# Baverne/VAE-CYCLEGAN-Implementation

Hardware: AMD Instinct MI355X
Metric: train images/sec (256x256 VAE-CycleGAN step) (higher is better)
Workload: dtype f32; 1 GPU; cyclevaegan unpaired, 3x256x256 synthetic summer<->winter, per-GPU batch 8, latent 64 (BASELINE.json configs[3]/[4]); per_gpu_batch=8, global_batch=8, image_size=256, latent_dim=64, parallelism=dp1, init=random (reference init statistics)

## Files before the change

vae-cyclegan-implementation_amd/csrc/conv_igemm.hip:

```cpp
#include "vcg_common.h"
#ifdef VCG_STAMP
#include <stdlib.h>
#endif

struct ConvP {
  const float* a;
  const float* b;
  const float* bias;
  float* out;
  int N, H, W, Cin, Cout, KH, KW, stride, pad, reflect, ups, act;
  int Hl, Wl, Ho, Wo, M, K;
  int cin4, cout4, cout_log;
  FastDiv fd_howo, fd_wo, fd_cin4, fd_cout4, fd_kw, fd_cin;
  int Hc, Wc, Mc, NB;
  FastDiv fd_hcwc, fd_wc;
  int ktiles_total, sk_len, sk_units, sk_ntn, sk_bm_shift, sk_bn_shift;
  int sk_ntr_pb;
  FastDiv fd_sklen;
  int ksplit, kt_per;
  float* slab;
  int adjoint;
  int src_pitch;
  uint32_t a_bytes, b_bytes;
  int dbl_mirror;
// ... 1891 lines not shown
typedef void (*ConvKernel)(ConvP);
struct KernelRef { ConvKernel fn; const char* name; };

static KernelRef fwd_fp32_kernel(const Tile& t, bool single_level) {
  const char* const name = "k_conv_fwd<fp32 MFMA>";
  if (t.bm == 128 && t.bn == 128 && single_level) return {k_conv_fwd<128, 128, 2, false>, name};
  if (t.bn == 32) return {k_conv_fwd<128, 32, 1>, name};
  if (t.bm == 128 && t.bn == 128) return {k_conv_fwd<128, 128>, name};
  if (t.bm == 128 && t.bn == 64) return {k_conv_fwd<128, 64>, name};
  if (t.bm == 64 && t.bn == 128) return {k_conv_fwd<64, 128>, name};
  return {k_conv_fwd<64, 64>, name};
}
static void launch_fwd_tile(const Tile& t, const KernelRef& k, const ConvP& p, hipStream_t st) {
  dim3 grid((p.M + t.bm - 1) / t.bm, (p.Cout + t.bn - 1) / t.bn, p.nbatch * p.ksplit);
  VcgProfScope prof(k.name, 2.0 * p.M * (double)p.K * p.Cout * p.nbatch, st);
  hipLaunchKernelGGL(k.fn, grid, dim3(256), 0, st, p);
}

static ConvGeom gemm_geom(int rows, int K, int Ncols) {
  ConvGeom g = {};
  g.N = 1; g.H = 1; g.W = rows; g.Cin = K; g.Cout = Ncols; g.KH = g.KW = 1; g.stride = 1; g.pad = 0; g.reflect = 0;
  g.ups = 1; g.act = VCG_ACT_NONE; g.cin_log = K; g.cout_log = Ncols;
  g.Hl = 1; g.Wl = rows; g.Ho = 1; g.Wo = rows; g.M = rows; g.K = K; g.taps = 1;
  return g;
}
int vcg_gemm_batched(const float* A, const float* B, float* C, int rows, int K, int Ncols, int batches, hipStream_t st) {
  ConvP p; fill_params(gemm_geom(rows, K, Ncols), p);
  p.a = A; p.b = B; p.bias = nullptr; p.out = C;
  if (set_extents(p, (unsigned long long)rows * K * 4, (unsigned long long)K * Ncols * 4,
                  "vcg_gemm_batched: operand extents must stay below 2 GiB per batch")) return -1;
  p.nbatch = batches; p.a_bstride = (uint32_t)((size_t)rows * K); p.b_bstride = (uint32_t)((size_t)K * Ncols);
  p.out_bstride = (size_t)rows * Ncols;
  VCG_CHECK_ARG((unsigned long long)rows * K * (unsigned long long)batches < (1ull << 32), "vcg_gemm_batched: batch stride overflow");
  const Tile t = gemm_plan(rows, Ncols, (K + BK - 1) / BK, false, batches, false, K <= 2048);
  launch_fwd_tile(t, fwd_fp32_kernel(t, K <= 2048), p, st);
  VCG_LAUNCH_CHECK("vcg_gemm_batched");
  return 0;
}

int vcg_fwd_launch(const ConvGeom& g, const float* x, const float* wf, float* y, hipStream_t st) {
  ConvP p; fill_params(g, p);
  p.a = x; p.b = wf; p.bias = nullptr; p.out = y; p.act = VCG_ACT_NONE;
  if (set_extents(p, (unsigned long long)g.N * g.H * g.W * g.Cin * 4, (unsigned long long)g.K * g.Cout * 4,
                  "vcg_conv_fwd: tensor extents must stay below 2 GiB")) return -1;
  const Tile t = gemm_plan(g.M, g.Cout, (g.K + BK - 1) / BK, false, 1, true);
  launch_fwd_tile(t, fwd_fp32_kernel(t, false), p, st);
  VCG_LAUNCH_CHECK("vcg_conv_fwd(raw)");
  return 0;
}

extern "C" size_t vcg_pack_weight_floats(const int32_t* cd) {
  ConvGeom g;
  if (vcg_conv_geom(cd, &g, "vcg_pack_weight_floats")) return 0;
  return pack_layout(g).total;
}

extern "C" int vcg_pack_weight(const float* w_oihw, float* wf, const int32_t* cd, void* stream) {
  ConvGeom g;
  if (vcg_conv_geom(cd, &g, "vcg_pack_weight")) return -1;
  VCG_CHECK_ARG(w_oihw && wf, "vcg_pack_weight: null pointer");
  const PackLayout L = pack_layout(g);
  hipStream_t st = (hipStream_t)stream;
  const VcgAmaxOut aw = vcg_amax_new(st);
  if (vcg_absmax_launch(w_oihw, (size_t)g.cout_log * g.cin_log * g.ups * g.ups * g.KH * g.KW, aw, st)) return -2;
  const VcgAmax amax_w = vcg_amax_in(aw);
  ConvP p; fill_params(g, p);
  p.amax_b = amax_w;
  if (L.wkd > L.wk && vcg_thin_fold_pack(g, w_oihw, wf + L.wk, amax_w, st)) return -2;
  if (L.wft > L.wkd && vcg_thin_fold_dgrad_pack(g, w_oihw, wf + L.wkd, amax_w, st)) return -2;
  if (L.wfd > L.wft) {
    const size_t tot = (size_t)g.Cout * ((g.K + 31) / 32) * 8;
    int blocks = (int)((tot + 255) / 256); if (blocks > 8192) blocks = 8192;
    hipLaunchKernelGGL(k_pack_planes<false>, dim3(blocks), dim3(256), 0, st, w_oihw, (unsigned short*)(wf + L.wft), p, g.cin_log,
                       g.cout_log);
    VCG_LAUNCH_CHECK("vcg_pack_weight(WFT planes)");
  }
  if (L.hdr > L.wfd) {
    const size_t tot = (size_t)g.K * (g.Cout / 4);
    int blocks = (int)((tot + 255) / 256); if (blocks > 8192) blocks = 8192;
    hipLaunchKernelGGL(k_pack_planes<true>, dim3(blocks), dim3(256), 0, st, w_oihw, (unsigned short*)(wf + L.wfd), p, g.cin_log,
                       g.cout_log);
    VCG_LAUNCH_CHECK("vcg_pack_weight(WFD planes)");
  }
  if (L.ud > L.u && vcg_wino_weight(g, w_oihw, wf + L.u, amax_w, st)) return -2;
  if (L.wk > L.ud && vcg_wino_weight_dgrad(g, w_oihw, wf + L.ud, amax_w, st)) return -2;
  uint32_t* const hdr = (uint32_t*)(wf + L.hdr);
  if (cd[VCG_CD_PACK_FLAGS] & 1) {
    ConvP q = p; q.K = 0; q.Cout = 0;
    hipLaunchKernelGGL(k_pack_weight, dim3(1), dim3(64), 0, st, w_oihw, wf, q, g.cin_log, g.cout_log, hdr);
    VCG_LAUNCH_CHECK("vcg_pack_weight(header)");
    return 0;
  }
  size_t total = (size_t)g.K * g.Cout;
  const size_t lds = (size_t)g.taps * 8 * 33 * sizeof(float);
  if (total < (1u << 20) || lds > 64 * 1024) {
    int blocks = (int)((total + 255) / 256); if (blocks > 4096) blocks = 4096;
    hipLaunchKernelGGL(k_pack_weight, dim3(blocks), dim3(256), 0, st, w_oihw, wf, p, g.cin_log, g.cout_log, hdr);
  } else {
    hipLaunchKernelGGL(k_pack_weight_t, dim3((g.Cout + 31) / 32, (g.Cin + 7) / 8), dim3(256), lds, st, w_oihw, wf, p, g.cin_log,
                       g.cout_log, hdr);
  }
  VCG_LAUNCH_CHECK("vcg_pack_weight");
  return 0;
}

static int ew_grid(size_t work) {
  size_t b = (work + 255) / 256;
  if (b > 2048) b = 2048;
  return b < 1 ? 1 : (int)b;
}

static KernelRef fwd_kernel(const FwdPlan& pl) {
  if (pl.path == FWD_FP32) return fwd_fp32_kernel(pl.t, pl.single_level);
  if (pl.t.bn == 128) return {k_conv_fwd_split<128>, "k_conv_fwd_split<128>"};
  return {k_conv_fwd_split<64>, "k_conv_fwd_split<64>"};
}

static uint64_t take_fwd_hints() {
  const uint64_t x_handle = vcg_take_hint_x(); (void)vcg_take_hint_dy();
  return x_handle;
}

static int conv_fwd_impl(const ConvGeom& g, const FwdPlan& pl, uint64_t x_handle, const float* x, const float* wf, const float* bias,
                         float* y, void* ws, size_t ws_bytes, void* stream, double* in_part, const VcgInStatsOut* stats,
                         float* saved = nullptr, const VcgPre* pre = nullptr) {
  VCG_CHECK_ARG(x && wf && y, "vcg_conv_fwd: null pointer");
  if (pre && pre->mean)
    VCG_CHECK_ARG(pl.pre_ok, "vcg_conv_fwd_in_pre: this geometry has no normalising gather (ask vcg_conv_pre_ok first)");
  const PackLayout L = pack_layout(g);
  const void* const w_amax = wf + L.hdr;
  hipStream_t st = (hipStream_t)stream;
  auto finalize = [&]() {
    return in_part ? vcg_in_finalize(in_part, stats->mean, stats->rstd, g.N, stats->HW, g.Cout, pl.stats_nchunk, stats->eps, st) : 0;
  };
  if (pl.path == FWD_THIN_FOLD) return vcg_thin_fold_fwd(g, x, wf + L.wk, w_amax, bias, y, ws, ws_bytes, st, x_handle);
  if (pl.path == FWD_THIN) return vcg_thin_fwd(g, x, wf, bias, y, st);
  if (pl.path == FWD_THININ) return vcg_thinin_fwd(g, x, wf, w_amax, bias, y, in_part, st, x_handle) ? -2 : finalize();
  if (pl.path == FWD_WINO) return vcg_wino_fwd(g, x, wf + L.u, w_amax, bias, y, ws, ws_bytes, st, in_part, stats, saved, x_handle, pre);
  if (pl.path == FWD_SLAB) return vcg_slab_fwd(g, x, wf + L.wft, (L.wfd - L.wft) * 4, w_amax, bias, y, in_part, stats, st, x_handle);
  ConvP p; fill_params(g, p);
  if (in_part) { p.in_part = in_part; p.in_nchunk = pl.stats_nchunk; }
  p.a = x; p.b = wf; p.bias = bias; p.out = y;
  if (set_extents(p, (unsigned long long)g.N * g.H * g.W * g.Cin * 4, (unsigned long long)g.K * g.Cout * 4,
                  "vcg_conv_fwd: tensor extents must stay below 2 GiB")) return -1;
  const int nsplit = pl.t.nsplit;
  if (nsplit > 1) {
    VCG_CHECK_ARG(ws && ws_bytes >= pl.ws, "vcg_conv_fwd: workspace too small (%zu)", ws_bytes);
    p.ksplit = nsplit; p.kt_per = pl.t.kt_per; p.slab = (float*)ws;
  }
  if (pl.path == FWD_SPLIT) {
    p.b = wf + L.wft;
    p.b_bytes = (uint32_t)((L.wfd - L.wft) * 4);
    if (vcg_operand_amax(x, (size_t)g.N * g.H * g.W * g.Cin, x_handle, 0, st, &p.amax_a)) return -2;
    p.amax_b = vcg_amax_stored(w_amax);
  }
  launch_fwd_tile(pl.t, fwd_kernel(pl), p, st);
  if (nsplit > 1)
    hipLaunchKernelGGL(k_splitk_finish, dim3(ew_grid((size_t)g.M * g.Cout / 4)), dim3(256), 0, st, (const float*)ws, bias,
                       y, (size_t)g.M, g.Cout, nsplit, g.cout_log, g.act);
  VCG_LAUNCH_CHECK("vcg_conv_fwd");
  return finalize();
}

extern "C" size_t vcg_conv_fwd_workspace(const int32_t* cd) {
  ConvGeom g;
  if (vcg_conv_geom(cd, &g, "vcg_conv_fwd_workspace")) return 0;
  return plan_fwd(g).ws;
}
// ... 375 lines not shown
```

vae-cyclegan-implementation_amd/csrc/conv_wino.hip:

```cpp
#include "vcg_common.h"
#ifdef VCG_STAMP
#include <stdlib.h>
#endif

#define WINO_U_SHIFT 2
#define WINO_V_SHIFT 2
int vcg_gemm_planes_batched(const void* APlanes, const void* BtPlanes, float* C, int rows, int K, int N, int batches, const VcgAmax& amax_a,
                            const VcgAmax& amax_b, hipStream_t st, uint32_t* amax_a_keep);

struct WinoP {
  const float* x;
  const float* m;
  const float* bias;
  float* y;
  int N, H, W, Cin, Cout, Hl, Wl, ups, reflect, act, cout_log;
  int th, tw, T, Kc;
  int off;
  FastDiv fd_k4, fd_tw, fd_thtw, fd_c4, fd_co4;
  unsigned long long* amax_slot;
  uint32_t amax_gen;
  VcgAmax amax_x;
  unsigned short* vplanes;
  const float* pre_mean;
  const float* pre_rstd;
// ... 120 lines not shown
        }
      }
  }
}

__global__ __launch_bounds__(256) void k_wino_out_stats(WinoP p, double* __restrict__ part, NormPlan pl) {
  __shared__ double r1[256 * 4];
  __shared__ double r2[256 * 4];
  const int tc = threadIdx.x % pl.TC, tp = threadIdx.x / pl.TC;
  const int c4 = blockIdx.z * pl.TC + tc;
  const int n = blockIdx.y;
  const int tiles = p.th * p.tw;
  const int pb = blockIdx.x * pl.chunk;
  int pe = pb + pl.chunk;
  if (pe > tiles) pe = tiles;
  const size_t plane = (size_t)p.T * p.Cout;
  double s1[4] = {0.0, 0.0, 0.0, 0.0}, s2[4] = {0.0, 0.0, 0.0, 0.0};
  if (c4 * 4 < p.Cout) {
    const int co = c4 * 4;
    float4 bv = make_float4(0.f, 0.f, 0.f, 0.f);
    if (p.bias) {
      if (co + 0 < p.cout_log) bv.x = p.bias[co + 0];
      if (co + 1 < p.cout_log) bv.y = p.bias[co + 1];
      if (co + 2 < p.cout_log) bv.z = p.bias[co + 2];
      if (co + 3 < p.cout_log) bv.w = p.bias[co + 3];
    }
    for (int tl = pb + tp; tl < pe; tl += pl.TP) {
      const int ty = tl / p.tw, tx = tl - ty * p.tw;
      const size_t t = (size_t)n * tiles + tl;
      const float* mb = p.m + t * p.Cout + co;
      float4 a0[4], a1[4];
#pragma unroll
      for (int b = 0; b < 4; ++b) {
        const float4 m0 = *reinterpret_cast<const float4*>(mb + (size_t)(0 + b) * plane);
        const float4 m1 = *reinterpret_cast<const float4*>(mb + (size_t)(4 + b) * plane);
        const float4 m2 = *reinterpret_cast<const float4*>(mb + (size_t)(8 + b) * plane);
        const float4 m3 = *reinterpret_cast<const float4*>(mb + (size_t)(12 + b) * plane);
        a0[b] = f4sum(f4sum(m0, m1), m2);
        a1[b] = f4sub(f4sub(m1, m2), m3);
      }
      float4 y[2][2];
      y[0][0] = f4sum(f4sum(a0[0], a0[1]), a0[2]);
      y[0][1] = f4sub(f4sub(a0[1], a0[2]), a0[3]);
      y[1][0] = f4sum(f4sum(a1[0], a1[1]), a1[2]);
      y[1][1] = f4sub(f4sub(a1[1], a1[2]), a1[3]);
#pragma unroll
      for (int r = 0; r < 2; ++r)
#pragma unroll
        for (int q = 0; q < 2; ++q) {
          float4 o = y[r][q];
          o.x = act_apply(o.x + bv.x, p.act); o.y = act_apply(o.y + bv.y, p.act);
          o.z = act_apply(o.z + bv.z, p.act); o.w = act_apply(o.w + bv.w, p.act);
          *reinterpret_cast<float4*>(p.y + (((size_t)n * p.Hl + 2 * ty + r) * p.Wl + 2 * tx + q) * p.Cout + co) = o;
          s1[0] += (double)o.x; s2[0] += (double)o.x * (double)o.x;
          s1[1] += (double)o.y; s2[1] += (double)o.y * (double)o.y;
          s1[2] += (double)o.z; s2[2] += (double)o.z * (double)o.z;
          s1[3] += (double)o.w; s2[3] += (double)o.w * (double)o.w;
        }
    }
  }
#pragma unroll
  for (int e = 0; e < 4; ++e) {
    r1[threadIdx.x * 4 + e] = s1[e];
    r2[threadIdx.x * 4 + e] = s2[e];
  }
  __syncthreads();
  if (tp == 0 && c4 * 4 < p.Cout) {
    for (int k = 1; k < pl.TP; ++k) {
#pragma unroll
      for (int e = 0; e < 4; ++e) {
        s1[e] += r1[(k * pl.TC + tc) * 4 + e];
        s2[e] += r2[(k * pl.TC + tc) * 4 + e];
      }
    }
    double* o = part + (((size_t)n * pl.nchunk + blockIdx.x) * p.Cout + c4 * 4) * 2;
#pragma unroll
    for (int e = 0; e < 4; ++e) {
      o[2 * e] = s1[e];
      o[2 * e + 1] = s2[e];
    }
  }
}

template <bool DGRAD>
__global__ __launch_bounds__(256) void k_wino_weight_planes(const float* __restrict__ w, unsigned short* __restrict__ up, int Cin,
                                                            int Cout, int ups, int cin_log, int cout_log, VcgAmax amax) {
  float sc, inv;
  vcg_scale_of(vcg_amax_bits(amax), amax.shift, sc, inv);
  const int U2 = ups * ups, Kc = U2 * Cin;
  const int NR = DGRAD ? Kc : Cout, KD = DGRAD ? Cout : Kc;
  const size_t total = (size_t)NR * (KD / 4);
  for (size_t idx = (size_t)blockIdx.x * blockDim.x + threadIdx.x; idx < total; idx += (size_t)gridDim.x * blockDim.x) {
    const int n = (int)(idx / (KD / 4)), kk = (int)(idx - (size_t)n * (KD / 4)) * 4;
    float t[16][4];
#pragma unroll
    for (int e = 0; e < 4; ++e) {
      const int co = DGRAD ? kk + e : n, k = DGRAD ? n : kk + e;
      const int ph = k / Cin, c = k - ph * Cin;
      const bool ok = co < cout_log && c < cin_log;
      const float* wp = w + ((size_t)co * (cin_log * U2) + (size_t)c * U2 + ph) * 9;
      float g[3][3];
#pragma unroll
      for (int a = 0; a < 3; ++a)
#pragma unroll
        for (int b = 0; b < 3; ++b) g[a][b] = ok ? (DGRAD ? wp[(2 - a) * 3 + (2 - b)] : wp[a * 3 + b]) : 0.f;
      float h[4][3];
#pragma unroll
      for (int b = 0; b < 3; ++b) {
        h[0][b] = g[0][b];
        h[1][b] = 0.5f * (g[0][b] + g[1][b] + g[2][b]);
        h[2][b] = 0.5f * (g[0][b] - g[1][b] + g[2][b]);
        h[3][b] = g[2][b];
      }
#pragma unroll
      for (int a = 0; a < 4; ++a) {
        t[a * 4 + 0][e] = h[a][0];
        t[a * 4 + 1][e] = 0.5f * (h[a][0] + h[a][1] + h[a][2]);
        t[a * 4 + 2][e] = 0.5f * (h[a][0] - h[a][1] + h[a][2]);
        t[a * 4 + 3][e] = h[a][2];
      }
    }
#pragma unroll
    for (int xi = 0; xi < 16; ++xi) {
      uint2 hh, ll;
      split4h(make_float4(t[xi][0], t[xi][1], t[xi][2], t[xi][3]), inv, hh, ll);
      unsigned short* o = up + (((size_t)xi * NR + n) * (KD / 32) + kk / 32) * VCG_PBLK + (kk & 31);
      *reinterpret_cast<uint2*>(o) = hh;
      *reinterpret_cast<uint2*>(o + 32) = ll;
    }
  }
}

__global__ __launch_bounds__(256) void k_wino_out_pad(const float* __restrict__ m, float* __restrict__ dxp, WinoP p) {
  const uint32_t k4n = (uint32_t)p.Kc / 4;
  const size_t total = (size_t)p.T * k4n;
  const size_t plane = (size_t)p.T * p.Kc;
  const int Hp = 2 * p.th, Wp = 2 * p.tw;
  for (size_t idx = (size_t)blockIdx.x * blockDim.x + threadIdx.x; idx < total; idx += (size_t)gridDim.x * blockDim.x) {
    const uint32_t t = (uint32_t)(idx / k4n);
    const int k = (int)(idx - (size_t)t * k4n) * 4;
    const uint32_t n = fd_div(t, p.fd_thtw);
    const uint32_t rem = t - n * (uint32_t)(p.th * p.tw);
    const uint32_t ty = fd_div(rem, p.fd_tw);
    const int tx = (int)(rem - ty * (uint32_t)p.tw);
    const float* mb = m + (size_t)t * p.Kc + k;
    float4 s0[4], s1[4];
#pragma unroll
    for (int b = 0; b < 4; ++b) {
      const float4 m0 = *reinterpret_cast<const float4*>(mb + (size_t)(0 + b) * plane);
      const float4 m1 = *reinterpret_cast<const float4*>(mb + (size_t)(4 + b) * plane);
      const float4 m2 = *reinterpret_cast<const float4*>(mb + (size_t)(8 + b) * plane);
      const float4 m3 = *reinterpret_cast<const float4*>(mb + (size_t)(12 + b) * plane);
      s0[b] = f4sum(f4sum(m0, m1), m2);
      s1[b] = f4sub(f4sub(m1, m2), m3);
    }
    float* o = dxp + (((size_t)n * Hp + 2 * ty) * Wp + 2 * tx) * p.Kc + k;
    *reinterpret_cast<float4*>(o) = f4sum(f4sum(s0[0], s0[1]), s0[2]);
    *reinterpret_cast<float4*>(o + p.Kc) = f4sub(f4sub(s0[1], s0[2]), s0[3]);
    *reinterpret_cast<float4*>(o + (size_t)Wp * p.Kc) = f4sum(f4sum(s1[0], s1[1]), s1[2]);
    *reinterpret_cast<float4*>(o + (size_t)Wp * p.Kc + p.Kc) = f4sub(f4sub(s1[1], s1[2]), s1[3]);
  }
}

__device__ __forceinline__ float4 wino_out_elem(const float* __restrict__ mb, size_t plane, int rr, int cc) {
  float4 acc = make_float4(0.f, 0.f, 0.f, 0.f);
#pragma unroll
  for (int i = 0; i < 3; ++i) {
    const int xi_r = rr + i;
    const float sr = (rr == 1 && i > 0) ? -1.f : 1.f;
#pragma unroll
    for (int j = 0; j < 3; ++j) {
      const int xi_c = cc + j;
      const float sc = (cc == 1 && j > 0) ? -1.f : 1.f;
      const float4 v = *reinterpret_cast<const float4*>(mb + (size_t)(xi_r * 4 + xi_c) * plane);
      const float sg = sr * sc;
      acc.x += sg * v.x; acc.y += sg * v.y; acc.z += sg * v.z; acc.w += sg * v.w;
    }
  }
  return acc;
}
__global__ __launch_bounds__(256) void k_wino_out_fold(const float* __restrict__ m, float* __restrict__ dx, WinoP p, int Hl, int Wl,
                                                       int Cin, int ups, int reflect) {
  const uint32_t k4n = (uint32_t)p.Kc / 4;
  const size_t total = (size_t)p.T * k4n;
  const size_t plane = (size_t)p.T * p.Kc;
  const int W = Wl * ups;
  for (size_t idx = (size_t)blockIdx.x * blockDim.x + threadIdx.x; idx < total; idx += (size_t)gridDim.x * blockDim.x) {
    const uint32_t t = (uint32_t)(idx / k4n);
    const int k = (int)(idx - (size_t)t * k4n) * 4;
    const uint32_t n = fd_div(t, p.fd_thtw);
    const uint32_t rem = t - n * (uint32_t)(p.th * p.tw);
    const int ty = (int)fd_div(rem, p.fd_tw);
    const int tx = (int)(rem - (uint32_t)ty * (uint32_t)p.tw);
    const float* mb = m + (size_t)t * p.Kc + k;
    float4 s0[4], s1[4];
#pragma unroll
    for (int b = 0; b < 4; ++b) {
      const float4 m0 = *reinterpret_cast<const float4*>(mb + (size_t)(0 + b) * plane);
      const float4 m1 = *reinterpret_cast<const float4*>(mb + (size_t)(4 + b) * plane);
      const float4 m2 = *reinterpret_cast<const float4*>(mb + (size_t)(8 + b) * plane);
      const float4 m3 = *reinterpret_cast<const float4*>(mb + (size_t)(12 + b) * plane);
      s0[b] = f4sum(f4sum(m0, m1), m2);
      s1[b] = f4sub(f4sub(m1, m2), m3);
    }
    float4 o[2][2];
    o[0][0] = f4sum(f4sum(s0[0], s0[1]), s0[2]);
    o[0][1] = f4sub(f4sub(s0[1], s0[2]), s0[3]);
    o[1][0] = f4sum(f4sum(s1[0], s1[1]), s1[2]);
    o[1][1] = f4sub(f4sub(s1[1], s1[2]), s1[3]);
    const int ph = k / Cin, c = k - ph * Cin;
    const int pi = ph >> 1, pj = ph & 1;
// ... 167 lines not shown
    e[2][s] = f4sub(d[2][s], d[1][s]);
    e[3][s] = f4sub(d[1][s], d[3][s]);
  }
  const uint32_t k = k4 * 4;
  const size_t KB = (size_t)p.Kc / 32;
  const int TB = p.T / 32;
#pragma unroll
  for (int a = 0; a < 4; ++a) {
    const float4 o[4] = {f4sub(e[a][0], e[a][2]), f4sum(e[a][1], e[a][2]), f4sub(e[a][2], e[a][1]), f4sub(e[a][1], e[a][3])};
    if (p.vplanes) {
      unsigned short* vb = p.vplanes + ((size_t)t * KB + k / 32) * VCG_PBLK + (k & 31);
      const size_t plane = (size_t)p.T * KB * VCG_PBLK;
#pragma unroll
      for (int b = 0; b < 4; ++b) {
        uint2 h, l;
        split4h(o[b], inv, h, l);
        unsigned short* w = vb + (size_t)(a * 4 + b) * plane;
        *reinterpret_cast<uint2*>(w) = h;
        *reinterpret_cast<uint2*>(w + 32) = l;
      }
    }
    if (vt) wino_tr_store(sh, o, inv, tl, q, vt + (size_t)(a * 4) * p.Kc * TB * VCG_PBLK, (size_t)p.Kc * TB * VCG_PBLK, (size_t)blockIdx.y * 32, TB, (int)blockIdx.x);
  }
}
__global__ __launch_bounds__(256) void k_wino_dy_tr(const float* __restrict__ dy, unsigned short* __restrict__ dmt, WinoP p) {
  __shared__ __attribute__((aligned(16))) unsigned short sh[4 * 2 * 32 * WT_PITCH];
  float sc, inv;
  vcg_scale_of(vcg_amax_bits(p.amax_x), p.amax_x.shift, sc, inv);
  const int tl = threadIdx.x >> 3, q = threadIdx.x & 7;
  const uint32_t t = blockIdx.x * 32 + tl;
  const int co = ((int)blockIdx.y * 8 + q) * 4;
  const uint32_t n = fd_div(t, p.fd_thtw);
  const uint32_t rem = t - n * (uint32_t)(p.th * p.tw);
  const uint32_t ty = fd_div(rem, p.fd_tw);
  const int tx = (int)(rem - ty * (uint32_t)p.tw);
  const float* base = dy + (((size_t)n * p.Hl + 2 * ty) * p.Wl + 2 * tx) * p.Cout + co;
  const float4 y00 = *reinterpret_cast<const float4*>(base);
  const float4 y01 = *reinterpret_cast<const float4*>(base + p.Cout);
  const float4 y10 = *reinterpret_cast<const float4*>(base + (size_t)p.Wl * p.Cout);
  const float4 y11 = *reinterpret_cast<const float4*>(base + (size_t)p.Wl * p.Cout + p.Cout);
  const float4 zero = make_float4(0.f, 0.f, 0.f, 0.f);
  float4 z[4][2];
  z[0][0] = y00;              z[0][1] = y01;
  z[1][0] = f4sum(y00, y10);  z[1][1] = f4sum(y01, y11);
  z[2][0] = f4sub(y00, y10);  z[2][1] = f4sub(y01, y11);
  z[3][0] = f4sub(zero, y10); z[3][1] = f4sub(zero, y11);
  const int TB = p.T / 32;
#pragma unroll
  for (int a = 0; a < 4; ++a) {
    const float4 o[4] = {z[a][0], f4sum(z[a][0], z[a][1]), f4sub(z[a][0], z[a][1]), f4sub(zero, z[a][1])};
    wino_tr_store(sh, o, inv, tl, q, dmt + (size_t)(a * 4) * p.Cout * TB * VCG_PBLK, (size_t)p.Cout * TB * VCG_PBLK, (size_t)blockIdx.y * 32, TB, (int)blockIdx.x);
  }
}

static int wino_blocks(size_t work) {
  size_t b = (work + 255) / 256;
  if (b > 8192) b = 8192;
  return b < 1 ? 1 : (int)b;
}

bool vcg_wino_weight_ok(const ConvGeom& g) {
  return g.KH == 3 && g.KW == 3 && g.stride == 1 && g.pad == 1 && g.ups * g.ups * g.Cin >= 128 && g.Cout >= 64 &&
         g.Cin % 4 == 0 && g.Cout % 64 == 0 && (g.ups * g.ups * g.Cin) % 64 == 0;
}
static bool wino_map_ok(const ConvGeom& g) {
  if (!vcg_wino_weight_ok(g)) return false;
#ifdef VCG_STAMP
  if (getenv("VCG_NO_WINOGRAD")) return false;
#endif
  return !(g.Ho < 4 || g.Wo < 4 || (g.Ho & 1) || (g.Wo & 1));
}
bool vcg_wino_fwd_ok(const ConvGeom& g) {
  if (!wino_map_ok(g)) return false;
  const unsigned long long T = (unsigned long long)g.N * (g.Ho / 2) * (g.Wo / 2);
  const unsigned long long Kc = (unsigned long long)g.ups * g.ups * g.Cin;
  if (Kc * g.Cout < (unsigned long long)kWinoGateFwd * (Kc + g.Cout)) return false;
  return T * Kc * 4 < (1ull << 31) && T * g.Cout * 4 < (1ull << 31) && T * Kc * 16 < (1ull << 32);
}
size_t vcg_wino_weight_floats(const ConvGeom& g) { return (size_t)16 * g.ups * g.ups * g.Cin * g.Cout * VCG_NP / 2; }
size_t vcg_wino_fwd_workspace(const ConvGeom& g) {
  const size_t T = (size_t)g.N * (g.Ho / 2) * (g.Wo / 2);
  return (size_t)16 * T * ((size_t)g.ups * g.ups * g.Cin + g.Cout) * sizeof(float) + 512;
}
int vcg_wino_weight(const ConvGeom& g, const float* w_oihw, float* u, const VcgAmax& amax_w, hipStream_t st) {
  const size_t total = (size_t)g.ups * g.ups * g.Cin * g.Cout / 4;
  VcgAmax au = amax_w; au.shift += WINO_U_SHIFT;
  hipLaunchKernelGGL(k_wino_weight_planes<false>, dim3(wino_blocks(total)), dim3(256), 0, st, w_oihw, (unsigned short*)u, g.Cin, g.Cout,
                     g.ups, g.cin_log, g.cout_log, au);
  VCG_LAUNCH_CHECK("vcg_wino_weight");
  return 0;
}

static WinoP wino_params(const ConvGeom& g) {
  WinoP p = {};
  p.x = nullptr; p.m = nullptr; p.bias = nullptr; p.y = nullptr;
  p.N = g.N; p.H = g.H; p.W = g.W; p.Cin = g.Cin; p.Cout = g.Cout; p.Hl = g.Hl; p.Wl = g.Wl; p.ups = g.ups;
  p.reflect = g.reflect; p.act = g.act; p.cout_log = g.cout_log;
  p.th = g.Ho / 2; p.tw = g.Wo / 2; p.T = g.N * p.th * p.tw; p.Kc = g.ups * g.ups * g.Cin;
  p.fd_k4 = make_fastdiv((uint32_t)p.Kc / 4); p.fd_tw = make_fastdiv((uint32_t)p.tw);
  p.fd_thtw = make_fastdiv((uint32_t)(p.th * p.tw)); p.fd_c4 = make_fastdiv((uint32_t)g.Cin / 4);
  p.fd_co4 = make_fastdiv((uint32_t)g.Cout / 4);
  p.off = 1;
  p.amax_slot = nullptr; p.amax_gen = 0;
  p.amax_x = vcg_amax_const(0); p.vplanes = nullptr;
  p.pre_mean = nullptr; p.pre_rstd = nullptr; p.pre_act = VCG_ACT_NONE;
  return p;
}

bool vcg_wino_wgrad_ok(const ConvGeom& g) {
  const long long kc = (long long)g.ups * g.ups * g.Cin;
  return vcg_wino_fwd_ok(g) && kc % 128 == 0 && kc * g.Cout >= kWinoGateWgrad * (kc + g.Cout);
}
bool vcg_wino_wgrad_tr_ok(const ConvGeom& g) {
  if (!vcg_wino_wgrad_ok(g)) return false;
  const long long kc = (long long)g.ups * g.ups * g.Cin, T = (long long)g.N * (g.Ho / 2) * (g.Wo / 2);
  return T % 32 == 0 && kc % 32 == 0 && g.Cout % 128 == 0 && kc >= 256 && ((kc + 255) / 256) * (g.Cout / 128) * 16 >= 192 &&
         16 * kc * T * VCG_NP < (1ll << 32) && 16 * (long long)g.Cout * T * VCG_NP < (1ll << 32);
}
size_t vcg_wino_wgrad_workspace(const ConvGeom& g) {
  const int T = g.N * (g.Ho / 2) * (g.Wo / 2);
  return vcg_wino_fwd_workspace(g) + vcg_wino_wgrad_core_workspace(g, T);
}
static size_t wino_v_floats(const ConvGeom& g) { return (size_t)16 * g.N * (g.Ho / 2) * (g.Wo / 2) * g.ups * g.ups * g.Cin; }
size_t vcg_wino_saved_floats(const ConvGeom& g) { return vcg_wino_wgrad_ok(g) ? wino_v_floats(g) + 16 : 0; }
int vcg_wino_wgrad(const ConvGeom& g, const float* x, const float* dy, float* gw_oihw, void* ws, size_t ws_bytes, hipStream_t st,
                   const float* v_saved, uint64_t x_handle, uint64_t dy_handle) {
  VCG_CHECK_ARG(ws && ws_bytes >= vcg_wino_wgrad_workspace(g), "vcg_conv_wgrad: workspace too small for the Winograd path");
  WinoP p = wino_params(g);
  float* V = (float*)ws;
  float* dM = V + (((size_t)16 * p.T * p.Kc + 63) / 64) * 64;
  const size_t tbytes = vcg_wino_fwd_workspace(g);
  if (vcg_wino_wgrad_tr_ok(g)) {
    VcgAmax amax_v;
    const unsigned short* Vt;
    if (v_saved) {
      Vt = reinterpret_cast<const unsigned short*>(v_saved);
      amax_v = vcg_amax_stored(v_saved + wino_v_floats(g), WINO_V_SHIFT);
    } else {
      if (vcg_operand_amax(x, (size_t)g.N * g.H * g.W * g.Cin, x_handle, WINO_V_SHIFT, st, &amax_v)) return -2;
      p.x = x; p.amax_x = amax_v; p.vplanes = nullptr;
      hipLaunchKernelGGL(k_wino_in_tr, dim3(p.T / 32, p.Kc / 32), dim3(256), 0, st, p, (unsigned short*)V);
      Vt = reinterpret_cast<const unsigned short*>(V);
    }
    VcgAmax amax_d;
    if (vcg_operand_amax(dy, (size_t)g.N * g.Ho * g.Wo * g.Cout, dy_handle, WINO_V_SHIFT, st, &amax_d)) return -2;
    WinoP pd = p;
    pd.amax_x = amax_d;
    hipLaunchKernelGGL(k_wino_dy_tr, dim3(p.T / 32, g.Cout / 32), dim3(256), 0, st, dy, (unsigned short*)dM, pd);
    VCG_LAUNCH_CHECK("vcg_conv_wgrad(winograd transforms, transposed)");
    float* dU = reinterpret_cast<float*>((char*)ws + tbytes);
    if (vcg_gemm_planes_batched(Vt, dM, dU, p.Kc, p.T, g.Cout, 16, amax_v, amax_d, st, nullptr)) return -2;
    return vcg_wino_wgrad_reduce_one(g, dU, gw_oihw, st);
  }
  p.x = x;
  VcgAmax amax_v;
  if (v_saved) {
    V = const_cast<float*>(v_saved);
    amax_v = vcg_amax_stored(v_saved + wino_v_floats(g), WINO_V_SHIFT);
  } else {
    if (vcg_operand_amax(x, (size_t)g.N * g.H * g.W * g.Cin, x_handle, WINO_V_SHIFT, st, &amax_v)) return -2;
    p.amax_x = amax_v; p.vplanes = (unsigned short*)V;
    hipLaunchKernelGGL(k_wino_in_planes, dim3(wino_blocks((size_t)p.T * p.Kc / 4)), dim3(256), 0, st, p);
  }
  const VcgAmaxOut ad = vcg_amax_new(st);
  p.amax_slot = ad.slot; p.amax_gen = ad.gen;
  hipLaunchKernelGGL(k_wino_dy, dim3(wino_blocks((size_t)p.T * g.Cout / 4)), dim3(256), 0, st, dy, dM, p);
  VCG_LAUNCH_CHECK("vcg_conv_wgrad(winograd transforms)");
  return vcg_wino_wgrad_core(g, V, dM, p.T, gw_oihw, (char*)ws + tbytes, ws_bytes - tbytes, st, amax_v, vcg_amax_in(ad));
}

bool vcg_wino_dgrad_ok(const ConvGeom& g) {
  if (!wino_map_ok(g)) return false;
  const long long kc = (long long)g.ups * g.ups * g.Cin;
  if (kc * g.Cout < kWinoGateDgrad * (kc + g.Cout)) return false;
  const unsigned long long Tp = (unsigned long long)g.N * (g.Ho / 2 + 1) * (g.Wo / 2 + 1);
  return Tp * kc * 4 < (1ull << 31) && Tp * g.Cout * 4 < (1ull << 31) && Tp * g.Cout * 16 < (1ull << 32);
}
size_t vcg_wino_dgrad_workspace(const ConvGeom& g) {
  const size_t Tp = (size_t)g.N * (g.Ho / 2 + 1) * (g.Wo / 2 + 1);
  const size_t kc = (size_t)g.ups * g.ups * g.Cin;
  return (size_t)16 * Tp * (kc + g.Cout) * sizeof(float) + 1024;
}
int vcg_wino_weight_dgrad(const ConvGeom& g, const float* w_oihw, float* ud, const VcgAmax& amax_w, hipStream_t st) {
  const size_t total = (size_t)g.ups * g.ups * g.Cin * g.Cout / 4;
  VcgAmax au = amax_w; au.shift += WINO_U_SHIFT;
  hipLaunchKernelGGL(k_wino_weight_planes<true>, dim3(wino_blocks(total)), dim3(256), 0, st, w_oihw, (unsigned short*)ud, g.Cin, g.Cout,
                     g.ups, g.cin_log, g.cout_log, au);
  VCG_LAUNCH_CHECK("vcg_wino_weight_dgrad");
  return 0;
}
int vcg_wino_dgrad(const ConvGeom& g, const float* dy, const float* ud, const void* w_amax, float* dx, void* ws, size_t ws_bytes,
                   hipStream_t st, uint64_t dy_handle) {
  VCG_CHECK_ARG(ws && ws_bytes >= vcg_wino_dgrad_workspace(g), "vcg_conv_dgrad: workspace too small for the Winograd path");
  const int kc = g.ups * g.ups * g.Cin;
  WinoP p = {};
  p.x = dy; p.bias = nullptr; p.y = nullptr;
  p.N = g.N; p.H = g.Ho; p.W = g.Wo; p.Cin = g.Cout; p.Cout = kc; p.Hl = g.Ho; p.Wl = g.Wo; p.ups = 1;
  p.reflect = 0; p.act = VCG_ACT_NONE; p.cout_log = kc;
  p.th = g.Ho / 2 + 1; p.tw = g.Wo / 2 + 1; p.T = g.N * p.th * p.tw; p.Kc = g.Cout; p.off = 2;
  p.amax_slot = nullptr; p.amax_gen = 0;
  p.amax_x = vcg_amax_const(0); p.vplanes = nullptr;
  p.fd_k4 = make_fastdiv((uint32_t)p.Kc / 4); p.fd_tw = make_fastdiv((uint32_t)p.tw);
  p.fd_thtw = make_fastdiv((uint32_t)(p.th * p.tw)); p.fd_c4 = make_fastdiv((uint32_t)p.Cin / 4);
  p.fd_co4 = make_fastdiv((uint32_t)kc / 4);
  float* V = (float*)ws;
  float* M = V + (((size_t)16 * p.T * g.Cout + 63) / 64) * 64;
  p.m = M;
  VcgAmax ad;
  if (vcg_operand_amax(dy, (size_t)g.N * g.Ho * g.Wo * g.Cout, dy_handle, WINO_V_SHIFT, st, &ad)) return -2;
  p.amax_x = ad; p.vplanes = (unsigned short*)V;
  hipLaunchKernelGGL(k_wino_in_planes, dim3(wino_blocks((size_t)p.T * g.Cout / 4)), dim3(256), 0, st, p);
  VCG_LAUNCH_CHECK("vcg_conv_dgrad(winograd input transform)");
  if (vcg_gemm_planes_batched(V, ud, M, p.T, g.Cout, kc, 16, ad, vcg_amax_stored(w_amax, WINO_U_SHIFT), st, nullptr)) return -2;
  WinoP q = p;
  q.Kc = kc;
  hipLaunchKernelGGL(k_wino_out_fold, dim3(wino_blocks((size_t)p.T * kc / 4)), dim3(256), 0, st, (const float*)M, dx, q, g.Hl, g.Wl,
                     g.Cin, g.ups, g.reflect);
  VCG_LAUNCH_CHECK("vcg_conv_dgrad(winograd output transform)");
  return 0;
}

size_t vcg_wino_fwd_stats_doubles(const ConvGeom& g) {
  const NormPlan pl = vcg_norm_plan(g.N, (g.Ho / 2) * (g.Wo / 2), g.Cout);
  return (size_t)g.N * pl.nchunk * g.Cout * 2;
}
int vcg_wino_fwd(const ConvGeom& g, const float* x, const float* u, const void* w_amax, const float* bias, float* y, void* ws,
                 size_t ws_bytes, hipStream_t st, double* in_part, const VcgInStatsOut* stats, float* v_keep, uint64_t x_handle,
                 const VcgPre* pre) {
  VCG_CHECK_ARG(ws && ws_bytes >= vcg_wino_fwd_workspace(g), "vcg_conv_fwd: workspace too small for the Winograd path (%zu)",
                ws_bytes);
  WinoP p = wino_params(g);
  float* V = v_keep ? v_keep : (float*)ws;
  float* M = (float*)ws + (((size_t)16 * p.T * p.Kc + 63) / 64) * 64;
  p.x = x; p.m = M; p.bias = bias; p.y = y;
  uint32_t pre_bits = 0;
  if (pre && pre->mean) {
    p.pre_mean = pre->mean; p.pre_rstd = pre->rstd; p.pre_act = pre->act;
    const float bound = sqrtf((float)g.H * (float)g.W);
    memcpy(&pre_bits, &bound, 4);
  }
  uint32_t* const keep_word = v_keep ? reinterpret_cast<uint32_t*>(v_keep + wino_v_floats(g)) : nullptr;
  if (v_keep && vcg_wino_wgrad_tr_ok(g)) {
    VcgAmax ax;
    if (pre_bits) ax = vcg_amax_const(pre_bits, WINO_V_SHIFT);
    else if (vcg_operand_amax(x, (size_t)g.N * g.H * g.W * g.Cin, x_handle, WINO_V_SHIFT, st, &ax)) return -2;
    V = (float*)ws;
    p.amax_x = ax; p.vplanes = (unsigned short*)V;
    hipLaunchKernelGGL(k_wino_in_tr, dim3(p.T / 32, p.Kc / 32), dim3(256), 0, st, p, (unsigned short*)v_keep);
    VCG_LAUNCH_CHECK("vcg_conv_fwd(winograd input transform, + transposed)");
    if (vcg_gemm_planes_batched(V, u, M, p.T, p.Kc, g.Cout, 16, ax, vcg_amax_stored(w_amax, WINO_U_SHIFT), st, keep_word)) return -2;
  } else {
    VcgAmax ax;
    if (pre_bits) ax = vcg_amax_const(pre_bits, WINO_V_SHIFT);
    else if (vcg_operand_amax(x, (size_t)g.N * g.H * g.W * g.Cin, x_handle, WINO_V_SHIFT, st, &ax)) return -2;
    p.amax_x = ax; p.vplanes = (unsigned short*)V;
    hipLaunchKernelGGL(k_wino_in_planes, dim3(wino_blocks((size_t)p.T * p.Kc / 4)), dim3(256), 0, st, p);
    VCG_LAUNCH_CHECK("vcg_conv_fwd(winograd input transform)");
    if (vcg_gemm_planes_batched(V, u, M, p.T, p.Kc, g.Cout, 16, ax, vcg_amax_stored(w_amax, WINO_U_SHIFT), st, keep_word)) return -2;
  }
  if (in_part) {
    const NormPlan pl = vcg_norm_plan(g.N, p.th * p.tw, g.Cout);
    hipLaunchKernelGGL(k_wino_out_stats, dim3(pl.nchunk, g.N, pl.cgroups), dim3(256), 0, st, p, in_part, pl);
    VCG_LAUNCH_CHECK("vcg_conv_fwd(winograd output transform)");
    return vcg_in_finalize(in_part, stats->mean, stats->rstd, g.N, stats->HW, g.Cout, pl.nchunk, stats->eps, st);
  } else {
    hipLaunchKernelGGL(k_wino_out, dim3(wino_blocks((size_t)p.T * g.Cout / 4)), dim3(256), 0, st, p);
  }
  VCG_LAUNCH_CHECK("vcg_conv_fwd(winograd output transform)");
  return 0;
}
```

vae-cyclegan-implementation_amd/csrc/vcg_common.h:

```cpp
#pragma once
#include <hip/hip_runtime.h>
#include <stdint.h>
#include <stdio.h>
#include <string.h>
#include "../../include/vcg.h"

#define VCG_WAVE 64

typedef float f32x16 __attribute__((ext_vector_type(16)));
typedef float f32x4 __attribute__((ext_vector_type(4)));

void vcg_set_error(const char* fmt, ...);

#define VCG_CHECK_ARG(cond, ...)      \
  do {                                \
    if (!(cond)) {                    \
      vcg_set_error(__VA_ARGS__);     \
      return -1;                      \
    }                                 \
  } while (0)

#define VCG_LAUNCH_CHECK(name)                                              \
  do {                                                                      \
    hipError_t e__ = hipGetLastError();                                     \
// ... 141 lines not shown
__device__ __forceinline__ uint32_t vcg_abs_bits4(const float4& v) {
  const uint32_t a = vcg_abs_bits(v.x), b = vcg_abs_bits(v.y), c = vcg_abs_bits(v.z), d = vcg_abs_bits(v.w);
  const uint32_t ab = a > b ? a : b, cd = c > d ? c : d;
  return ab > cd ? ab : cd;
}
__device__ __forceinline__ uint32_t vcg_amax_bits(const VcgAmax& a) {
  if (!a.slot) return a.stored ? *a.stored : a.bits;
  const unsigned long long w = a.slot[threadIdx.x & 63];
  uint32_t b = (uint32_t)(w >> 32) == a.gen ? (uint32_t)w : 0u;
#pragma unroll
  for (int o = 32; o > 0; o >>= 1) {
    const uint32_t other = (uint32_t)__shfl_xor((int)b, o, 64);
    b = other > b ? other : b;
  }
  return b;
}
#endif
__host__ __device__ static inline void vcg_scale_of(uint32_t amax_bits, int shift, float& s, float& inv) {
  int e = (int)((amax_bits >> 23) & 0xFF);
  int f = (e == 0 || e == 255) ? 127 + shift : e - 14 + shift;
  f = f < 1 ? 1 : (f > 253 ? 253 : f);
  const uint32_t sb = (uint32_t)f << 23, ib = (uint32_t)(254 - f) << 23;
#ifdef __HIP_DEVICE_COMPILE__
  s = __uint_as_float(sb); inv = __uint_as_float(ib);
#else
  memcpy(&s, &sb, 4); memcpy(&inv, &ib, 4);
#endif
}

struct NormPlan {
  int TC, TP, cgroups, nchunk, chunk;
};
static inline NormPlan vcg_norm_plan(int N, int HW, int C) {
  NormPlan pl;
  int c4 = C / 4;
  int tc = 1;
  while (tc * 2 <= c4 && tc * 2 <= 32) tc *= 2;
  pl.TC = tc;
  pl.TP = 256 / tc;
  pl.cgroups = (c4 + tc - 1) / tc;
  long long target = 1024 / ((long long)N * pl.cgroups);
  if (target < 1) target = 1;
  long long maxc = (HW + pl.TP * 2 - 1) / (pl.TP * 2);
  if (maxc < 1) maxc = 1;
  if (target > maxc) target = maxc;
  pl.chunk = (int)((HW + target - 1) / target);
  pl.nchunk = (HW + pl.chunk - 1) / pl.chunk;
  return pl;
}
int vcg_in_finalize(const double* part, float* mean, float* rstd, int N, int HW, int C, int nchunk, float eps, hipStream_t st);

struct VcgInStatsOut {
  float* mean;
  float* rstd;
  int HW;
  float eps;
};
int vcg_in_stats_pass(const float* t, float* mean, float* rstd, int N, int HW, int C, float eps, void* ws, size_t ws_bytes, hipStream_t st);

struct ConvGeom {
  int N, H, W, Cin, Cout, KH, KW, stride, pad, reflect, ups, act, cin_log, cout_log;
  int Hl, Wl, Ho, Wo, M, K, taps;
};

int vcg_conv_geom(const int32_t* cd, ConvGeom* g, const char* who);

bool vcg_thin_fwd_ok(const ConvGeom& g);
bool vcg_thin_dgrad_ok(const ConvGeom& g);
size_t vcg_thin_dgrad_workspace(const ConvGeom& g);
int vcg_thin_fwd(const ConvGeom& g, const float* x, const float* wf, const float* bias, float* y, hipStream_t st);
int vcg_thin_dgrad(const ConvGeom& g, const float* dy, const float* wf, float* dx, void* ws, size_t ws_bytes,
                   hipStream_t st);

bool vcg_thinin_fwd_ok(const ConvGeom& g);
int vcg_thinin_nchunk(const ConvGeom& g);
int vcg_thinin_fwd(const ConvGeom& g, const float* x, const float* wf, const void* w_amax, const float* bias, float* y, double* in_part,
                   hipStream_t st, uint64_t x_handle);

bool vcg_wino_weight_ok(const ConvGeom& g);
constexpr long long kWinoGateFwd = 100, kWinoGateDgrad = 80, kWinoGateWgrad = 128;
bool vcg_wino_fwd_ok(const ConvGeom& g);
size_t vcg_wino_weight_floats(const ConvGeom& g);
size_t vcg_wino_fwd_workspace(const ConvGeom& g);
int vcg_wino_weight(const ConvGeom& g, const float* w_oihw, float* u, const VcgAmax& amax_w, hipStream_t st);
struct VcgPre { const float* mean; const float* rstd; int act; };
int vcg_wino_fwd(const ConvGeom& g, const float* x, const float* u, const void* w_amax, const float* bias, float* y, void* ws,
                 size_t ws_bytes, hipStream_t st, double* in_part = nullptr, const VcgInStatsOut* stats = nullptr, float* v_keep = nullptr,
                 uint64_t x_handle = 0, const VcgPre* pre = nullptr);
size_t vcg_wino_saved_floats(const ConvGeom& g);
size_t vcg_wino_fwd_stats_doubles(const ConvGeom& g);
bool vcg_wino_wgrad_ok(const ConvGeom& g);
size_t vcg_wino_wgrad_workspace(const ConvGeom& g);
int vcg_wino_wgrad(const ConvGeom& g, const float* x, const float* dy, float* gw_oihw, void* ws, size_t ws_bytes, hipStream_t st,
                   const float* v_saved = nullptr, uint64_t x_handle = 0, uint64_t dy_handle = 0);
bool vcg_wino_wgrad_tr_ok(const ConvGeom& g);
int vcg_wino_wgrad_reduce_one(const ConvGeom& g, const float* dU, float* gw_oihw, hipStream_t st);
size_t vcg_wino_wgrad_core_workspace(const ConvGeom& g, int T);
int vcg_wino_wgrad_core(const ConvGeom& g, const float* V, const float* dM, int T, float* gw_oihw, void* ws, size_t ws_bytes,
                        hipStream_t st, const VcgAmax& amax_v, const VcgAmax& amax_dm);
bool vcg_wino_dgrad_ok(const ConvGeom& g);
size_t vcg_wino_dgrad_workspace(const ConvGeom& g);
int vcg_wino_weight_dgrad(const ConvGeom& g, const float* w_oihw, float* ud, const VcgAmax& amax_w, hipStream_t st);
int vcg_wino_dgrad(const ConvGeom& g, const float* dy, const float* ud, const void* w_amax, float* dx, void* ws, size_t ws_bytes,
                   hipStream_t st, uint64_t dy_handle = 0);
bool vcg_slab_fwd_ok(const ConvGeom& g);
bool vcg_slab_fwd_stats_ok(const ConvGeom& g);
int vcg_slab_fwd_nchunk(const ConvGeom& g);
bool vcg_slab_dgrad_ok(const ConvGeom& g);
size_t vcg_slab_dgrad_workspace(const ConvGeom& g);
int vcg_slab_fwd(const ConvGeom& g, const float* x, const void* wft_planes, size_t planes_bytes, const void* w_amax, const float* bias,
                 float* y, double* in_part, const VcgInStatsOut* stats, hipStream_t st, uint64_t x_handle = 0);
int vcg_slab_dgrad(const ConvGeom& g, const float* dy, const void* wfd_planes, size_t planes_bytes, const void* w_amax, float* dx,
                   void* ws, size_t ws_bytes, hipStream_t st, uint64_t dy_handle = 0);
bool vcg_ring_wgrad_ok(const ConvGeom& g);
size_t vcg_ring_wgrad_workspace(const ConvGeom& g);
int vcg_ring_wgrad(const ConvGeom& g, const float* x, const float* dy, float* gw_oihw, void* ws, size_t ws_bytes, hipStream_t st,
                   uint64_t x_handle = 0, uint64_t dy_handle = 0);
bool vcg_thin_fold_ok(const ConvGeom& g);
size_t vcg_thin_fold_weight_floats(const ConvGeom& g);
size_t vcg_thin_fold_workspace(const ConvGeom& g);
int vcg_thin_fold_pack(const ConvGeom& g, const float* w_oihw, float* wk, const VcgAmax& amax_w, hipStream_t st);
int vcg_thin_fold_fwd(const ConvGeom& g, const float* x, const float* wk, const void* w_amax, const float* bias, float* y, void* ws,
                      size_t ws_bytes, hipStream_t st, uint64_t x_handle = 0);
bool vcg_thin_fold_dgrad_ok(const ConvGeom& g);
size_t vcg_thin_fold_dgrad_weight_floats(const ConvGeom& g);
size_t vcg_thin_fold_dgrad_workspace(const ConvGeom& g);
int vcg_thin_fold_dgrad_pack(const ConvGeom& g, const float* w_oihw, float* wk, const VcgAmax& amax_w, hipStream_t st);
int vcg_thin_fold_dgrad(const ConvGeom& g, const float* dy, const float* wkd, const void* w_amax, float* dx, void* ws, size_t ws_bytes,
                        hipStream_t st, uint64_t dy_handle = 0);
```

Baseline: 247.1 images/s.

## Fuse Winograd forward and dgrad weight packing into one LDS-tiled kernel

Replaces the two per-element Winograd weight-transform kernels (forward and flipped dgrad) with one tiled kernel. It stages a 32x32 (Cin x Cout) block of OIHW weights in shared memory through coalesced float4 loads, then emits both the forward and dgrad transformed planes from that tile. This removes one launch and one redundant strided read of the weights per layer per step, and replaces scattered global reads with coalesced ones. In exchange it uses larger blocks (512 threads for upsample layers) and a big shared-memory tile, and it assumes Cout is a multiple of 32.

```diff
diff --git a/vae-cyclegan-implementation_amd/csrc/conv_igemm.hip b/vae-cyclegan-implementation_amd/csrc/conv_igemm.hip
--- a/vae-cyclegan-implementation_amd/csrc/conv_igemm.hip
+++ b/vae-cyclegan-implementation_amd/csrc/conv_igemm.hip
@@ -1997,8 +1997,7 @@
                        g.cout_log);
     VCG_LAUNCH_CHECK("vcg_pack_weight(WFD planes)");
   }
-  if (L.ud > L.u && vcg_wino_weight(g, w_oihw, wf + L.u, amax_w, st)) return -2;
-  if (L.wk > L.ud && vcg_wino_weight_dgrad(g, w_oihw, wf + L.ud, amax_w, st)) return -2;
+  if (L.wk > L.u && vcg_wino_weight(g, w_oihw, L.ud > L.u ? wf + L.u : nullptr, L.wk > L.ud ? wf + L.ud : nullptr, amax_w, st)) return -2;
   uint32_t* const hdr = (uint32_t*)(wf + L.hdr);
   if (cd[VCG_CD_PACK_FLAGS] & 1) {
     ConvP q = p; q.K = 0; q.Cout = 0;
diff --git a/vae-cyclegan-implementation_amd/csrc/conv_wino.hip b/vae-cyclegan-implementation_amd/csrc/conv_wino.hip
--- a/vae-cyclegan-implementation_amd/csrc/conv_wino.hip
+++ b/vae-cyclegan-implementation_amd/csrc/conv_wino.hip
@@ -226,51 +226,111 @@
   }
 }
 
-template <bool DGRAD>
-__global__ __launch_bounds__(256) void k_wino_weight_planes(const float* __restrict__ w, unsigned short* __restrict__ up, int Cin,
-                                                            int Cout, int ups, int cin_log, int cout_log, VcgAmax amax) {
+enum { WINO_W_FWD = 1, WINO_W_DGRAD = 2 };
+__device__ __forceinline__ void wino_g_transform(const float (&g)[3][3], float (&t)[16][4], int e) {
+  float h[4][3];
+#pragma unroll
+  for (int b = 0; b < 3; ++b) {
+    h[0][b] = g[0][b];
+    h[1][b] = 0.5f * (g[0][b] + g[1][b] + g[2][b]);
+    h[2][b] = 0.5f * (g[0][b] - g[1][b] + g[2][b]);
+    h[3][b] = g[2][b];
+  }
+#pragma unroll
+  for (int a = 0; a < 4; ++a) {
+    t[a * 4 + 0][e] = h[a][0];
+    t[a * 4 + 1][e] = 0.5f * (h[a][0] + h[a][1] + h[a][2]);
+    t[a * 4 + 2][e] = 0.5f * (h[a][0] - h[a][1] + h[a][2]);
+    t[a * 4 + 3][e] = h[a][2];
+  }
+}
+__device__ __forceinline__ void wino_w_store(const float (&t)[16][4], float inv, unsigned short* o, size_t xi_stride) {
+#pragma unroll
+  for (int xi = 0; xi < 16; ++xi) {
+    uint2 hh, ll;
+    split4h(make_float4(t[xi][0], t[xi][1], t[xi][2], t[xi][3]), inv, hh, ll);
+    *reinterpret_cast<uint2*>(o + xi * xi_stride) = hh;
+    *reinterpret_cast<uint2*>(o + xi * xi_stride + 32) = ll;
+  }
+}
+template <int U2, int OUT>
+__global__ __launch_bounds__(U2 == 1 ? 256 : 512) void k_wino_weight_tile(const float* __restrict__ w, unsigned short* __restrict__ u,
+                                                                          unsigned short* __restrict__ ud, int Cin, int Cout, int cin_log,
+                                                                          int cout_log, VcgAmax amax) {
+  constexpr int NT = U2 == 1 ? 256 : 512;
+  constexpr int RUN = 32 * U2 * 9, ROW = RUN + 1;
+  constexpr int ITEMS = 32 * U2 * 8;
+  __shared__ float tile[32 * ROW];
   float sc, inv;
   vcg_scale_of(vcg_amax_bits(amax), amax.shift, sc, inv);
-  const int U2 = ups * ups, Kc = U2 * Cin;
-  const int NR = DGRAD ? Kc : Cout, KD = DGRAD ? Cout : Kc;
-  const size_t total = (size_t)NR * (KD / 4);
-  for (size_t idx = (size_t)blockIdx.x * blockDim.x + threadIdx.x; idx < total; idx += (size_t)gridDim.x * blockDim.x) {
-    const int n = (int)(idx / (KD / 4)), kk = (int)(idx - (size_t)n * (KD / 4)) * 4;
-    float t[16][4];
-#pragma unroll
-    for (int e = 0; e < 4; ++e) {
-      const int co = DGRAD ? kk + e : n, k = DGRAD ? n : kk + e;
-      const int ph = k / Cin, c = k - ph * Cin;
-      const bool ok = co < cout_log && c < cin_log;
-      const float* wp = w + ((size_t)co * (cin_log * U2) + (size_t)c * U2 + ph) * 9;
-      float g[3][3];
-#pragma unroll
-      for (int a = 0; a < 3; ++a)
-#pragma unroll
-        for (int b = 0; b < 3; ++b) g[a][b] = ok ? (DGRAD ? wp[(2 - a) * 3 + (2 - b)] : wp[a * 3 + b]) : 0.f;
-      float h[4][3];
-#pragma unroll
-      for (int b = 0; b < 3; ++b) {
-        h[0][b] = g[0][b];
-        h[1][b] = 0.5f * (g[0][b] + g[1][b] + g[2][b]);
-        h[2][b] = 0.5f * (g[0][b] - g[1][b] + g[2][b]);
-        h[3][b] = g[2][b];
-      }
-#pragma unroll
-      for (int a = 0; a < 4; ++a) {
-        t[a * 4 + 0][e] = h[a][0];
-        t[a * 4 + 1][e] = 0.5f * (h[a][0] + h[a][1] + h[a][2]);
-        t[a * 4 + 2][e] = 0.5f * (h[a][0] - h[a][1] + h[a][2]);
-        t[a * 4 + 3][e] = h[a][2];
-      }
-    }
-#pragma unroll
-    for (int xi = 0; xi < 16; ++xi) {
-      uint2 hh, ll;
-      split4h(make_float4(t[xi][0], t[xi][1], t[xi][2], t[xi][3]), inv, hh, ll);
-      unsigned short* o = up + (((size_t)xi * NR + n) * (KD / 32) + kk / 32) * VCG_PBLK + (kk & 31);
-      *reinterpret_cast<uint2*>(o) = hh;
-      *reinterpret_cast<uint2*>(o + 32) = ll;
+  const int tid = threadIdx.x;
+  const int c0 = blockIdx.x * 32, co0 = blockIdx.y * 32, Kc = U2 * Cin;
+  const int cv = cin_log - c0 < 32 ? cin_log - c0 : 32;
+  const int valid = cv > 0 ? cv * U2 * 9 : 0;
+  const size_t rs = (size_t)cin_log * U2 * 9;
+  const float* src = w + (size_t)co0 * rs + (size_t)c0 * U2 * 9;
+  if (((cin_log * U2) & 3) == 0) {
+    constexpr int R4 = RUN / 4, N4 = 32 * R4 / NT;
+    float4 v[N4];
+#pragma unroll
+    for (int j = 0; j < N4; ++j) {
+      const int i = tid + j * NT, r = i / R4, q = (i - r * R4) * 4;
+      v[j] = co0 + r < cout_log && q < valid ? *reinterpret_cast<const float4*>(src + (size_t)r * rs + q) : make_float4(0.f, 0.f, 0.f, 0.f);
+    }
+#pragma unroll
+    for (int j = 0; j < N4; ++j) {
+      const int i = tid + j * NT, r = i / R4, q = (i - r * R4) * 4;
+      float* d = tile + r * ROW + q;
+      d[0] = v[j].x; d[1] = v[j].y; d[2] = v[j].z; d[3] = v[j].w;
+    }
+  } else {
+    for (int i = tid; i < 32 * RUN; i += NT) {
+      const int r = i / RUN, q = i - r * RUN;
+      tile[r * ROW + q] = co0 + r < cout_log && q < valid ? src[(size_t)r * rs + q] : 0.f;
+    }
+  }
+  __syncthreads();
+  if (OUT & WINO_W_FWD) {
+#pragma unroll 1
+    for (int it = tid; it < ITEMS; it += NT) {
+      const int c4 = it & 7, ph = (it >> 3) % U2, col = it / (8 * U2);
+      const int c = c0 + c4 * 4;
+      if (c >= Cin) continue;
+      float t[16][4];
+#pragma unroll
+      for (int e = 0; e < 4; ++e) {
+        const float* gp = tile + col * ROW + ((c4 * 4 + e) * U2 + ph) * 9;
+        float g[3][3];
+#pragma unroll
+        for (int a = 0; a < 3; ++a)
+#pragma unroll
+          for (int b = 0; b < 3; ++b) g[a][b] = gp[a * 3 + b];
+        wino_g_transform(g, t, e);
+      }
+      const int k = ph * Cin + c;
+      wino_w_store(t, inv, u + ((size_t)(co0 + col) * (Kc / 32) + k / 32) * VCG_PBLK + (k & 31), (size_t)Cout * (Kc / 32) * VCG_PBLK);
+    }
+  }
+  if (OUT & WINO_W_DGRAD) {
+#pragma unroll 1
+    for (int it = tid; it < ITEMS; it += NT) {
+      const int co4 = it & 7, kl = it >> 3;
+      const int cl = kl / U2, ph = kl - cl * U2;
+      const int c = c0 + cl;
+      if (c >= Cin) continue;
+      float t[16][4];
+#pragma unroll
+      for (int e = 0; e < 4; ++e) {
+        const float* gp = tile + (co4 * 4 + e) * ROW + kl * 9;
+        float g[3][3];
+#pragma unroll
+        for (int a = 0; a < 3; ++a)
+#pragma unroll
+          for (int b = 0; b < 3; ++b) g[a][b] = gp[(2 - a) * 3 + (2 - b)];
+        wino_g_transform(g, t, e);
+      }
+      const int k = ph * Cin + c, co = co0 + co4 * 4;
+      wino_w_store(t, inv, ud + ((size_t)k * (Cout / 32) + co / 32) * VCG_PBLK + (co & 31), (size_t)Kc * (Cout / 32) * VCG_PBLK);
     }
   }
 }
@@ -604,11 +664,23 @@
   const size_t T = (size_t)g.N * (g.Ho / 2) * (g.Wo / 2);
   return (size_t)16 * T * ((size_t)g.ups * g.ups * g.Cin + g.Cout) * sizeof(float) + 512;
 }
-int vcg_wino_weight(const ConvGeom& g, const float* w_oihw, float* u, const VcgAmax& amax_w, hipStream_t st) {
-  const size_t total = (size_t)g.ups * g.ups * g.Cin * g.Cout / 4;
+template <int U2>
+static void wino_weight_launch(const ConvGeom& g, const float* w_oihw, unsigned short* u, unsigned short* ud, const VcgAmax& au,
+                               hipStream_t st) {
+  const dim3 grid((g.Cin + 31) / 32, g.Cout / 32), block(U2 == 1 ? 256 : 512);
+  if (u && ud)
+    hipLaunchKernelGGL((k_wino_weight_tile<U2, WINO_W_FWD | WINO_W_DGRAD>), grid, block, 0, st, w_oihw, u, ud, g.Cin, g.Cout, g.cin_log,
+                       g.cout_log, au);
+  else if (u)
+    hipLaunchKernelGGL((k_wino_weight_tile<U2, WINO_W_FWD>), grid, block, 0, st, w_oihw, u, ud, g.Cin, g.Cout, g.cin_log, g.cout_log, au);
+  else
+    hipLaunchKernelGGL((k_wino_weight_tile<U2, WINO_W_DGRAD>), grid, block, 0, st, w_oihw, u, ud, g.Cin, g.Cout, g.cin_log, g.cout_log, au);
+}
+int vcg_wino_weight(const ConvGeom& g, const float* w_oihw, float* u, float* ud, const VcgAmax& amax_w, hipStream_t st) {
+  VCG_CHECK_ARG((u || ud) && vcg_wino_weight_ok(g), "vcg_wino_weight: not a Winograd layer");
   VcgAmax au = amax_w; au.shift += WINO_U_SHIFT;
-  hipLaunchKernelGGL(k_wino_weight_planes<false>, dim3(wino_blocks(total)), dim3(256), 0, st, w_oihw, (unsigned short*)u, g.Cin, g.Cout,
-                     g.ups, g.cin_log, g.cout_log, au);
+  if (g.ups == 1) wino_weight_launch<1>(g, w_oihw, (unsigned short*)u, (unsigned short*)ud, au, st);
+  else wino_weight_launch<4>(g, w_oihw, (unsigned short*)u, (unsigned short*)ud, au, st);
   VCG_LAUNCH_CHECK("vcg_wino_weight");
   return 0;
 }
@@ -702,14 +774,6 @@
   const size_t Tp = (size_t)g.N * (g.Ho / 2 + 1) * (g.Wo / 2 + 1);
   const size_t kc = (size_t)g.ups * g.ups * g.Cin;
   return (size_t)16 * Tp * (kc + g.Cout) * sizeof(float) + 1024;
-}
-int vcg_wino_weight_dgrad(const ConvGeom& g, const float* w_oihw, float* ud, const VcgAmax& amax_w, hipStream_t st) {
-  const size_t total = (size_t)g.ups * g.ups * g.Cin * g.Cout / 4;
-  VcgAmax au = amax_w; au.shift += WINO_U_SHIFT;
-  hipLaunchKernelGGL(k_wino_weight_planes<true>, dim3(wino_blocks(total)), dim3(256), 0, st, w_oihw, (unsigned short*)ud, g.Cin, g.Cout,
-                     g.ups, g.cin_log, g.cout_log, au);
-  VCG_LAUNCH_CHECK("vcg_wino_weight_dgrad");
-  return 0;
 }
 int vcg_wino_dgrad(const ConvGeom& g, const float* dy, const float* ud, const void* w_amax, float* dx, void* ws, size_t ws_bytes,
                    hipStream_t st, uint64_t dy_handle) {
diff --git a/vae-cyclegan-implementation_amd/csrc/vcg_common.h b/vae-cyclegan-implementation_amd/csrc/vcg_common.h
--- a/vae-cyclegan-implementation_amd/csrc/vcg_common.h
+++ b/vae-cyclegan-implementation_amd/csrc/vcg_common.h
@@ -247,7 +247,7 @@
 bool vcg_wino_fwd_ok(const ConvGeom& g);
 size_t vcg_wino_weight_floats(const ConvGeom& g);
 size_t vcg_wino_fwd_workspace(const ConvGeom& g);
-int vcg_wino_weight(const ConvGeom& g, const float* w_oihw, float* u, const VcgAmax& amax_w, hipStream_t st);
+int vcg_wino_weight(const ConvGeom& g, const float* w_oihw, float* u, float* ud, const VcgAmax& amax_w, hipStream_t st);
 struct VcgPre { const float* mean; const float* rstd; int act; };
 int vcg_wino_fwd(const ConvGeom& g, const float* x, const float* u, const void* w_amax, const float* bias, float* y, void* ws,
                  size_t ws_bytes, hipStream_t st, double* in_part = nullptr, const VcgInStatsOut* stats = nullptr, float* v_keep = nullptr,
@@ -265,7 +265,6 @@
                         hipStream_t st, const VcgAmax& amax_v, const VcgAmax& amax_dm);
 bool vcg_wino_dgrad_ok(const ConvGeom& g);
 size_t vcg_wino_dgrad_workspace(const ConvGeom& g);
-int vcg_wino_weight_dgrad(const ConvGeom& g, const float* w_oihw, float* ud, const VcgAmax& amax_w, hipStream_t st);
 int vcg_wino_dgrad(const ConvGeom& g, const float* dy, const float* ud, const void* w_amax, float* dx, void* ws, size_t ws_bytes,
                    hipStream_t st, uint64_t dy_handle = 0);
 bool vcg_slab_fwd_ok(const ConvGeom& g);
```

After: 246.2 images/s. About the same (-0.4%).
